# gt1/daccord

Measured on AMD Instinct MI355X. Metric: corrected Mbase/s (whole node), synthetic 20x PacBio piles, higher is better.
Workload: dtype u64+f64; 1 GPU; BASELINE.json configs[1] (10k A-reads x 10 kb x 20x, k=14, one MI355X): synthetic 10000 A-reads x 10000 b x 20x, 15% error (ins 80/del 13.3/sub 6.7), k=14, w=40, a=10, tspace=100; piles_total=10000, piles_rank0=10000, overlaps_rank0=319252, windows_rank0=9969965, trace_blocks_rank0=17906701, corrected_bases_total=90715992

## Files before the change

### daccord_amd/csrc/capi.hip

```cpp
#include <hip/hip_runtime.h>
#include <vector>
#include <string>
#include <cstring>
#include <cstdio>
#include <cstdlib>
#include <new>
#include "../../include/daccord_hip.h"
#include "batch_plan.hpp"
#include "host_tables.hpp"
#include "window_kernels.hpp"
#include "trace_kernel.hpp"
#include "vote_kernel.hpp"
#include "emit_record.hpp"
#include "context.hpp"

using namespace dacc;


struct PrepBatch
{
	DevOvl const * ovl; uint64_t novl; uint8_t const * trace; uint32_t trace_bytes;
	uint32_t * blk_ovl; uint32_t * blk_b0;
};

// ... 296 lines not shown
}

int dacc_create(dacc_ctx ** out, dacc_params const * p)
{
	if ( !out || !p ) return DACC_EINVAL;
	*out = 0;
	if ( p->klow < 3 || p->khigh > 16 || p->klow > p->khigh || !p->w || !p->a || p->w > DACC_WMAX || p->minfilterfreq < 0 ||
	     p->maxfilterfreq < p->minfilterfreq || p->tspace <= 0 || p->tspace > 512 )
		return DACC_EINVAL;
	if ( readTierSwitches().conflict() ) return DACC_EINVAL;
	int ndev = 0;
	if ( hipGetDeviceCount(&ndev) != hipSuccess || ndev <= 0 || p->device < 0 || p->device >= ndev )
		return DACC_ENODEV;
	if ( hipSetDevice(p->device) != hipSuccess ) return DACC_ENODEV;
	dacc_ctx * c = new (std::nothrow) dacc_ctx;
	if ( !c ) return DACC_ENOMEM;
	c->par = *p; c->device = p->device;
	c->sw = readTierSwitches();
	char const * sc = getenv("DACC_SCHED"); c->env_sched = sc ? atoi(sc) : 1;
	{ char const * td = getenv("DACC_TRACE_DYN"); c->env_trdyn = !(td && td[0] == '0'); }
	char const * ta = getenv("DACC_T7_ADAPT"); c->env_t7adapt = !(ta && ta[0] == '0');
	char const * dr = getenv("DACC_DEBUG_RETRY"); c->env_dbgretry = (dr && dr[0] == '1');
	{ char const * fn = getenv("DACC_FEAS_NEED"); c->env_feasneed = (fn && fn[0] == '0') ? 0u : 1u; }
	if ( hipStreamCreate(&c->stream.h) != hipSuccess ) { delete c; return DACC_EHIP; }
	{ int lo = 0, hi = 0; hipDeviceGetStreamPriorityRange(&lo,&hi); if ( hipStreamCreateWithPriority(&c->stream2.h,hipStreamNonBlocking,hi) != hipSuccess ) { delete c; return DACC_EHIP; } }
	hipEventCreateWithFlags(&c->evFirstTier.h,hipEventDisableTiming); hipEventCreateWithFlags(&c->evEarlyGeneric.h,hipEventDisableTiming); hipEventCreateWithFlags(&c->evPrescan.h,hipEventDisableTiming);
	for ( Event & e : c->ev ) hipEventCreate(&e.h);
	for ( Event & e : c->evEmit ) hipEventCreate(&e.h);
	for ( Event & e : c->evLong ) hipEventCreate(&e.h);
	for ( Event & e : c->evslot ) hipEventCreate(&e.h);
	for ( dacc_ctx::Stage & S : c->st ) hipEventCreate(&S.done.h);
	hipEventCreate(&c->h2dend.h);
	*out = c;
	return DACC_OK;
}

void dacc_destroy(dacc_ctx * c)
{
	if ( !c ) return;
	hipSetDevice(c->device);
	hipStreamSynchronize(c->stream); hipStreamSynchronize(c->stream2);
	delete c;
}

char const * dacc_last_error(dacc_ctx * c) { return c ? c->err.c_str() : "null context"; }

// ... 71 lines not shown
static uint32_t * workCounter(dacc_ctx * c, uint32_t const off) { return (c->sched&1) ? c->d_work.p+off : static_cast<uint32_t *>(0); }
static dacc_ctx::Stage * ranOf(dacc_ctx * c, TierId const id) { return c->st[id].ran ? &c->st[id] : static_cast<dacc_ctx::Stage *>(0); }

struct Pass
{
	WindowBatch WB;
	uint32_t const * list = 0;
	int lastslot = -1;
	bool early = false;
	uint32_t herr[4] = {0,0,0,0};
	size_t symbytes = 0;
};

static WindowBatch windowBatch(dacc_ctx * c)
{
	BatchPlan & BP = c->BP; WindowBatch WB;
	WB.P = c->P; WB.T = c->T; WB.C = BP.caps; WB.bps = c->d_bps.p; WB.boff = c->d_boff.p; WB.rlen = c->d_rlen.p;
	WB.piles = c->d_piles.p; WB.npiles = BP.piles.size(); WB.ovl = c->d_ovl.p; WB.wt_b = c->d_wt_b.p; WB.wt_e = c->d_wt_e.p;
	WB.nwindows = BP.nwindows; WB.wrec = c->d_wrec.p; WB.wout = c->d_wout.p; WB.arena = c->d_arena.p; WB.prof = c->d_prof.p;
	return WB;
}
static FastBatch stageBatch(dacc_ctx * c, WindowBatch const & WB, uint32_t const id, bool const chain = true)
{
	FastBatch FB; FB.W = WB; FB.F = c->BP.stageCaps(id); FB.dpsq_vst = c->d_vst.p; FB.tab32 = c->d_tab32.p; FB.feasneed = c->env_feasneed;
	if ( !chain ) return FB;
	FB.hand = c->handcap ? c->d_hand.p : static_cast<uint64_t *>(0); FB.handctr = c->d_handctr.p; FB.handcap = c->handcap; FB.handwords = c->TP.handwords;
#if defined(DACC_LEDGER)
	{ char const * lm = getenv("DACC_LEDGER_MASK"); FB.ledger = lm ? static_cast<uint32_t>(strtoul(lm,0,0)) : 0u; }
#endif
	return FB;
}
static void handsOn(FastBatch & FB, uint32_t * const handon, uint8_t * const slab) { FB.retry = handon; FB.gslab = slab; FB.gstride = FB.F.gbytes; }

static void growHandOver(dacc_ctx * c)
{
	if ( !(c->nruns && c->handwant > c->handcap && !c->nohand) ) return;
	uint64_t cap = c->handwant;
	{ size_t fr = 0, tot = 0; if ( hipMemGetInfo(&fr,&tot) == hipSuccess ) { uint64_t const lim = (static_cast<uint64_t>(fr)/2) / (static_cast<uint64_t>(c->TP.handwords)*8ull); if ( cap > lim ) cap = lim; } else (void)hipGetLastError(); }
	while ( cap && c->d_hand.ensure(static_cast<size_t>(cap)*c->TP.handwords) != hipSuccess ) { (void)hipGetLastError(); cap = cap > 65536 ? cap/2 : 0; }
	c->handcap = static_cast<uint32_t>(cap); c->handwant = cap;
}

static int enqueuePrepAndTrace(dacc_ctx * c)
{
	BatchPlan & BP = c->BP; hipStream_t const s = c->stream;
	HIPCHK(hipMemsetAsync(c->d_err.p,0,4*sizeof(uint32_t),s));
	HIPCHK(hipEventRecord(c->ev[0],s));
// ... 682 lines not shown
```

### daccord_amd/csrc/context.hpp

```cpp
#ifndef DACC_CONTEXT_HPP
#define DACC_CONTEXT_HPP
#include <hip/hip_runtime.h>
#include <cstdlib>
#include <string>
#include <vector>
#include "../../include/daccord_hip.h"
#include "batch_plan.hpp"
#include "host_tables.hpp"
#include "window_main.hpp"
#include "vote_kernel.hpp"

namespace dacc {

template<typename T>
struct DevBuf
{
	T * p = 0; size_t cap = 0;
	DevBuf() = default; DevBuf(DevBuf const &) = delete; DevBuf & operator=(DevBuf const &) = delete;
	~DevBuf() { release(); }
	hipError_t ensure(size_t n)
	{
		if ( n <= cap ) return hipSuccess;
		if ( p ) { hipFree(p); p = 0; cap = 0; }
		hipError_t const e = hipMalloc(reinterpret_cast<void **>(&p),n*sizeof(T));
// ... 52 lines not shown
	DevBuf<uint8_t> d_bps; DevBuf<uint64_t> d_boff; DevBuf<uint32_t> d_rlen;
	std::vector<uint32_t> h_rlen;
	BatchPlan BP;
	DevBuf<DevPile> d_piles; DevBuf<DevOvl> d_ovl; DevBuf<uint32_t> d_ovl_pile; DevBuf<uint8_t> d_trace;
	DevBuf<uint32_t> d_blk_ovl, d_blk_b0, d_wt_b, d_wt_e;
	DevBuf<uint8_t> d_wrec; DevBuf<WindowOut> d_wout; DevBuf<uint8_t> d_arena;
	DevBuf<uint8_t> d_has, d_oc, d_outsym, d_pilebad; DevBuf<uint16_t> d_ld0; DevBuf<uint32_t> d_ocs, d_nfrag, d_err;
	DevBuf<VoteFragment> d_frags; DevBuf<uint64_t> d_fragbase; DevBuf<uint64_t> d_prof;
	DevBuf<uint64_t> d_vst; DevBuf<uint32_t> d_tab32; DevBuf<uint8_t> d_gslab, d_arena2; DevBuf<uint64_t> d_trslab;
	DevBuf<uint32_t> d_retry[TIER_NSLOTS], d_work, d_gearly, d_pregen, d_pregen2, d_pregenlist, d_small;
	DevBuf<uint8_t> d_longslab;
	DevBuf<uint32_t> d_longhand[2];
	DevBuf<uint64_t> d_hand; DevBuf<uint32_t> d_handctr; uint32_t handcap = 0; uint64_t handwant = 0, nruns = 0; bool nohand = false, oom = false;
	bool noslab = false;
	bool tier7_adapt_off = false;
	TierSwitches sw = {}; TierPipeline TP = {};
	struct Stage { bool ran = false; uint32_t grid = 0; DevBuf<uint32_t> handon; DevBuf<uint8_t> slab; Event done; uint32_t const * in = 0;  } st[TIER_NROWS];
	uint32_t nlong[2] = {0,0};
	bool longran[2] = {false,false}; Event evLong[4];
	uint32_t retry_grid = 0, early_grid = 0; int sched = 0;
	uint32_t tr_grid = 0, tr_lds = 0, tr_words = 0, tr_lanes = 0, trace_bytes = 0, win_grid = 0;
	int env_sched = 1, env_dbgretry = 0, env_t7adapt = 1, env_trdyn = 1;
	uint32_t env_feasneed = 1;
	std::vector<uint32_t> retry_flags;
	std::vector<dacc_fragment> frags; std::string bases;
	std::vector<int32_t> pile_status; std::vector<std::string> pile_errors; std::string pile_errors_joined;
	std::vector<uint32_t> h_nfrag; std::vector<VoteFragment> h_frags; HostBuf<uint8_t> h_outsym;
	dacc_timing timing = {};
};

}

struct dacc_ctx : dacc::Context {};
#endif
```

### daccord_amd/csrc/fast_window.hpp

```cpp
#ifndef DACC_FAST_WINDOW_HPP
#define DACC_FAST_WINDOW_HPP
#include "wave.hpp"
#include "dev_types.hpp"
#include "arena.hpp"
#include "window_main.hpp"
#include "tier_pipeline.hpp"
#include "emit_record.hpp"

namespace dacc {

enum { WS_RETRY = 4 };
enum { FNOPAR = 0xFF };
enum { FSEQCAP = 48 };

struct FSI { uint64_t w; uint16_t left, right, current, path; };
struct FCC { uint64_t w; uint32_t o, l; };

template<int TIER> struct FastTier;
#if !defined(DACC_RCH01)
#define DACC_RCH01 2
#endif
template<> struct FastTier<1> { typedef uint8_t id_t; typedef uint8_t sid_t; enum : uint32_t { smax = 250, gw = 1, wcapg = 1024, rch = DACC_RCH01, fch = 4, fnw = 2, fnc = 40, idmax = 250, rpstcap = 256, lstr = 64, maxs = 32, precap = 1024, ncap = 776, scap = 112, lcap = 960, wcap = 1024, rccap = 144, fcap = 192, siqcap = 56, blcap = 96, seqcap = 32, psiq = 8, consrow = 64, lscrids = 2048, wide = 0, mins = 0, gmem = 0 }; };
template<> struct FastTier<0> { typedef uint8_t id_t; typedef uint8_t sid_t; enum : uint32_t { smax = 250, gw = 1, wcapg = 768, rch = DACC_RCH01, fch = 4, fnw = 2, fnc = 32, idmax = 250, rpstcap = 256, lstr = 64, maxs = 28, precap = 576, ncap = 524, scap = 88, lcap = 640, wcap = 768, rccap = 96, fcap = 128, siqcap = 56, blcap = 96, seqcap = 32, psiq = 8, consrow = 64, lscrids = 2048, wide = 0, mins = 0, gmem = 0 }; };
template<> struct FastTier<7> { typedef uint8_t id_t; typedef uint8_t sid_t; enum : uint32_t { smax = 250, gw = 1, wcapg = 896, rch = DACC_RCH01, fch = 4, fnw = 2, fnc = 32, idmax = 250, rpstcap = 256, lstr = 64, maxs = 28, precap = 704, ncap = 640, scap = 104, lcap = 800, wcap = 896, rccap = 112, fcap = 148, siqcap = 56, blcap = 96, seqcap = 32, psiq = 8, consrow = 64, lscrids = 2048, wide = 0, mins = 0, gmem = 0 }; };
// ... 401 lines not shown
	C.fcap = CT::fcap; C.siqcap = CT::siqcap; C.blcap = CT::blcap;
	C.nrows = nrows; C.nsup = nsup;
	C.ldsbytes = FastLds<CT>::bytes(nrows,nsup);
	C.tabcap = FastLds<CT>::tabcap;
	if constexpr ( CT::gw != 0 ) C.gbytes = FastLds<CT>::g_total; else C.gbytes = 0;
	if constexpr ( FastOneSlab<CT>::value != 0 ) C.ldsbytes = C.gbytes;
	C.gmem = CT::gmem;
	static_assert(CT::gmem == 0 || CT::gw != 0,"a layout in device memory is the gw layout");
	return C;
}

struct FastBatch
{
	WindowBatch W;
	FastCaps F = {};
	uint64_t const * dpsq_vst = 0;
	uint32_t * retry = 0;
	uint32_t * gearly = 0;
	uint8_t * gslab = 0;
	uint64_t gstride = 0;
	uint32_t const * tab32 = 0;
	uint64_t * hand = 0; uint32_t * handctr = 0; uint32_t handcap = 0, handwords = 0;
	uint32_t feasneed = 1;
#if defined(DACC_LEDGER)
	uint32_t ledger = 0;
#endif
};

template<typename CT>
DEV void fast_load_tables(FastLds<CT> const & L, uint32_t const nrows, uint32_t const nsup, DevTables const & T, uint64_t const * vst)
{
	int const lane = wv_lane();
	for ( uint32_t i = lane; i < nsup; i += WSZ ) { L.suplo8()[i] = T.suplo[i]; L.suphi8()[i] = T.suphi[i]; }
	wv_sync();
}

#if defined(DACC_LEDGER)
#define LEDGER_REP(bit) for ( uint32_t lrep_ = 0, lrn_ = 1u + ((ledger >> (bit)) & 1u); lrep_ < lrn_; ++lrep_ )
#define LEDGER_REPX(E,bit) for ( uint32_t lrep_ = 0, lrn_ = 1u + (((E).ledger >> (bit)) & 1u); lrep_ < lrn_; ++lrep_ )
#else
#define LEDGER_REP(bit)
#define LEDGER_REPX(E,bit)
#endif
#define FW_THRES_FEAS 4294968ull
#define FW_THRES_01   429496730ull
#define FW_THRES_05   2147483648ull

#if defined(DACC_EMUL)
struct FastStats { uint32_t v[32]; void clear() { for ( int i = 0; i < 32; ++i ) v[i] = 0; } void mx(int i, uint32_t x) { if ( x > v[i] ) v[i] = x; } void add(int i, uint32_t x) { v[i] += x; } };
static FastStats g_fstats;
static inline void fstats_dump(int const tier)
{
	static FILE * sf = 0; static bool tried = false;
	if ( !tried ) { tried = true; char const * fn = getenv("DACC_EMUL_STATS"); if ( fn ) sf = fopen(fn,"w"); }
	if ( sf ) { fprintf(sf,"%d",tier); for ( int i = 0; i < 32; ++i ) fprintf(sf," %u",g_fstats.v[i]); fprintf(sf,"\n"); fflush(sf); }
}
static inline FILE * ftrav_file() { static FILE * f = 0; static bool tried = false; if ( !tried ) { tried = true; char const * fn = getenv("DACC_EMUL_TRAV"); if ( fn ) f = fopen(fn,"w"); } return f; }
#define FSTAT_MX(i,x) g_fstats.mx(i,x)
#define FSTAT_ADD(i,x) g_fstats.add(i,x)
#include <vector>
#include <algorithm>
struct FeasIters { std::vector<uint32_t> it, ln; void clear() { it.clear(); ln.clear(); } };
static FeasIters g_feasit;
static inline void feasit_dump()
{
	static FILE * f = 0; static bool tried = false;
	if ( !tried ) { tried = true; char const * fn = getenv("DACC_EMUL_FEAS"); if ( fn ) f = fopen(fn,"w"); }
	if ( !f ) { g_feasit.clear(); return; }
	std::vector<uint32_t> const & it = g_feasit.it; std::vector<uint32_t> const & ln = g_feasit.ln;
	uint64_t tot = 0, lock = 0, locksorted = 0;
	for ( size_t i = 0; i < it.size(); ++i ) tot += it[i];
	for ( size_t i = 0; i < it.size(); i += 64 ) { uint32_t m = 0; for ( size_t q = i; q < it.size() && q < i+64; ++q ) m = std::max(m,it[q]); lock += m; }
	std::vector< std::pair<uint32_t,uint32_t> > P; for ( size_t i = 0; i < it.size(); ++i ) P.push_back(std::make_pair(ln[i],it[i]));
	std::stable_sort(P.begin(),P.end(),[](std::pair<uint32_t,uint32_t> const & a, std::pair<uint32_t,uint32_t> const & b){ return a.first > b.first; });
	for ( size_t i = 0; i < P.size(); i += 64 ) { uint32_t m = 0; for ( size_t q = i; q < P.size() && q < i+64; ++q ) m = std::max(m,P[q].second); locksorted += m; }
	uint64_t lockcls = 0;
	{
		std::vector< std::pair<uint32_t,uint32_t> > Q; for ( size_t i = 0; i < it.size(); ++i ) { uint32_t c = 0; while ( (2u<<c) <= ln[i] ) ++c; Q.push_back(std::make_pair(c,it[i])); }
// ... 111 lines not shown
template<typename CT>
struct FastEngine
{
	typedef typename CT::id_t id_t;
	typedef typename CT::sid_t sid_t;
	enum : uint32_t { SB = 8u*sizeof(sid_t), SMASK = (1u<<SB)-1u, SNONE = SMASK, SMAX = CT::smax };
	FastLds<CT> L; DevTables T; DevParams P;
	uint32_t nrows, nsup;
	uint64_t const * vst;
	enum : bool { GW = (CT::gw != 0) };
	uint8_t * gslab;
	uint32_t const * gtab;
	struct G4 { uint32_t x, y, z, w; };
	int lane; uint32_t flags;
#if defined(DACC_LEDGER)
	uint32_t ledger;
#endif
	uint64_t * prof;
	uint32_t mao, k; uint64_t kmask;
	uint32_t npre, nlast, nn, nmfirst, nmlast;
	uint32_t n0, npool, nlinks, nwF, nwR;
	uint32_t nF, nL;
	uint32_t feasneed;

#if defined(DACC_EMUL)
	bool feascount, feasapplied; uint32_t nwFall, nwRall;
	DEV bool feasNeedOn() const { char const * e = getenv("DACC_FEAS_NEED"); return !(e && e[0] == '0'); }
#else
	static constexpr bool feascount = false;
	DEV bool feasNeedOn() const { return feasneed != 0; }
#endif
#if defined(DACC_EMUL)
	DEV void over_(uint32_t b, int line) { flags |= b; static char const * ov = getenv("DACC_EMUL_OVER"); if ( ov ) fprintf(stderr,"[over] tier maxs=%d line %d bits 0x%x nn=%u n0=%u npool=%u nF=%u nL=%u nwF=%u nwR=%u rstop=%u\n",int(CT::maxs)*10000+int(CT::ncap),line,b,nn,n0,npool,nF,nL,nwF,nwR,rstop); }
	#define over(b) over_(b,__LINE__)
#else
	DEV void over(uint32_t b) { flags |= b; }
#endif
#if defined(DACC_PROFILE) && !defined(DACC_EMUL)
	DEV void pcount(int id, uint64_t v) { if ( prof ) atomicAdd(reinterpret_cast<unsigned long long *>(prof+id),static_cast<unsigned long long>(v)); }
	DEV uint64_t pclock() { return clock64(); }
#else
	DEV void pcount(int, uint64_t) {}
	DEV uint64_t pclock() { return 0; }
#endif

#if defined(DACC_PROFILE) && !defined(DACC_EMUL)
	#define SITE_T0 uint64_t _ps = clock64();
	#define SITE_RESET { _ps = clock64(); }
	#define SITE(id) { uint64_t const _n = clock64(); if ( prof && lane == static_cast<int>(__builtin_ctzll(__builtin_amdgcn_ballot_w64(true))) ) { atomicAdd(reinterpret_cast<unsigned long long *>(prof+32+(id)),static_cast<unsigned long long>(_n-_ps)); atomicAdd(reinterpret_cast<unsigned long long *>(prof+80+(id)),1ull); } _ps = clock64(); }
	#define PROFX_T0 uint64_t _px = clock64();
	#define PROFX(id) { uint64_t const _n = clock64(); if ( lane == 0 && prof ) atomicAdd(reinterpret_cast<unsigned long long *>(prof+(id)),static_cast<unsigned long long>(_n-_px)); _px = _n; }
#else
	#define PROFX_T0
// ... 594 lines not shown
			L.tlast()[q] = static_cast<uint32_t>(sk);
		}
		wv_sync();
		uint32_t const p2 = next_pow2(ns < 2 ? 2 : ns);
		for ( uint32_t q = lane; q < p2; q += WSZ )
		{
			if constexpr ( KEY2 ) L.skey()[q] = q < ns ? ((((static_cast<uint64_t>(L.tfirst()[q])<<KF) | L.links()[L.tlink()[q]+1])<<QB) | q) : ~0ull;
			else
			L.skey()[q] = q < ns ? ((sortKey(L.tfirst()[q],L.links()[L.tlink()[q]+1],L.tslen()[q] < KFMAX ? L.tslen()[q] : KFMAX,L.tlast()[q])<<QB) | q) : ~0ull;
		}
		wv_sync();
		wv_sort_keys<fcpow2(CT::scap)>(L.skey(),ns);
		uint32_t dup = 0;
		for ( uint32_t q = lane; q < ns; q += WSZ )
		{
			enum : uint32_t { DUPSH = KEY2 ? QB : QB+2*KF };
			if ( q && (L.skey()[q]>>DUPSH) == (L.skey()[q-1]>>DUPSH) ) dup = 1;
			uint32_t const raw = L.skey()[q]&QMASK;
			L.sfirst()[q] = L.tfirst()[raw]; L.slast()[q] = L.tlast()[raw]; L.sslen()[q] = L.tslen()[raw]; L.slink()[q] = L.tlink()[raw];
		}
		if ( wv_any(dup) ) { over(32); n0 = 0; return; }
		n0 = ns;
		wv_sync();
		for ( uint32_t z = lane; z < nn; z += WSZ ) { L.npred()[z] = SNONE; L.lhead()[z] = SNONE; }
		for ( uint32_t q = lane; q < p2; q += WSZ ) L.skey()[q] = q < ns ? ((static_cast<uint64_t>(L.slast()[q])<<SB) | q) : ~0ull;
		wv_sync();
		for ( uint32_t q = lane; q < ns; q += WSZ ) if ( q == 0 || L.sfirst()[q-1] != L.sfirst()[q] ) L.npred()[L.sfirst()[q]] = q;
		wv_sort_keys<fcpow2(CT::scap)>(L.skey(),ns);
		for ( uint32_t q = lane; q < ns; q += WSZ )
		{
			uint64_t const e = L.skey()[q];
			L.lord()[q] = static_cast<uint32_t>(e);
			if ( q == 0 || (L.skey()[q-1]>>SB) != (e>>SB) ) L.lhead()[e>>SB] = q;
		}
		wv_sync();
	}

	DEV void makePiece(uint32_t const id, uint32_t const par, uint32_t const a, uint32_t const b)
	{
		LDSQ uint16_t const * Lk = L.links() + L.slink()[par];
		L.sfirst()[id] = Lk[a]; L.slast()[id] = Lk[b]; L.sslen()[id] = b-a+1; L.slink()[id] = L.slink()[par]+a;
	}
	DEV void findCandidatesAndPieces()
	{
		uint32_t const firstthres = nmfirst ? ((static_cast<uint32_t>((~L.mfirst()[0])>>32))*3)/4 : 0;
		uint32_t const lastthres = nmlast ? ((static_cast<uint32_t>((~L.mlast()[0])>>32))*3)/4 : 0;
		uint32_t cf = 0, cl = 0;
		while ( cf < nmfirst && static_cast<uint32_t>((~L.mfirst()[cf])>>32) >= firstthres ) ++cf;
		while ( cl < nmlast && static_cast<uint32_t>((~L.mlast()[cl])>>32) >= lastthres ) ++cl;
		nF = cf; npool = n0;
		if ( nF > FNC ) { nL = cl; over(8); return; }
		for ( uint32_t i = lane; i < nF; i += WSZ ) { uint32_t const km = static_cast<uint32_t>(~L.mfirst()[i]); L.fkmer()[i] = km; int32_t const z = findNode(km); L.fnode()[i] = z < 0 ? 0xFFFF : z; L.parF()[i] = SNONE; L.pieF()[i] = SNONE; }
		{
			uint32_t nl = 0;
			for ( uint32_t c = 0; c < cl; c += WSZ )
			{
				uint32_t const i = c + lane;
				uint32_t const km = i < cl ? static_cast<uint32_t>(~L.mlast()[i]) : 0u;
// ... 14 lines not shown
			for ( uint32_t z = lane; z < nn; z += WSZ ) sid[z] = 0xFFFF;
			wv_sync();
			for ( uint32_t s = lane; s < n0; s += WSZ )
			{
				uint32_t const len = L.sslen()[s]; LDSQ uint16_t const * Lk = L.links() + L.slink()[s];
				for ( uint32_t i = len > 2 ? len-2 : 0; i >= 1; --i ) { uint32_t const z = Lk[i]; sid[z] = s; spos[z] = i; }
			}
			wv_sync();
			for ( uint32_t s = lane; s < n0; s += WSZ )
			{
				uint32_t const len = L.sslen()[s]; LDSQ uint16_t const * Lk = L.links() + L.slink()[s];
				for ( uint32_t i = 1; i+1 < len; ++i ) if ( sid[Lk[i]] != s ) multi = 1;
			}
			for ( uint32_t c = lane; c < nF; c += WSZ ) { uint32_t const z = L.fnode()[c]; if ( z != 0xFFFF && sid[z] != 0xFFFF ) { L.parF()[c] = sid[z]; L.posF()[c] = spos[z]; } }
			for ( uint32_t c = lane; c < nL; c += WSZ ) { uint32_t const z = L.lnode()[c]; if ( z != 0xFFFF && sid[z] != 0xFFFF ) { L.parL()[c] = sid[z]; L.posL()[c] = spos[z]; } }
		}
		if ( wv_any(multi) ) { over(32); return; }
		wv_sync();
		{
			uint32_t cnt = 0;
			for ( uint32_t c = 0; c < nF; ++c ) cnt += (L.parF()[c] != SNONE);
			for ( uint32_t c = 0; c < nL; ++c ) cnt += (L.parL()[c] != SNONE);
			if ( n0 + 2*cnt + 1 > CT::scap || n0 + 2*cnt + 1 > SMAX ) { over(32); return; }
		}
		{
			uint32_t id = n0;
			for ( uint32_t c0 = 0; c0 < nF + nL; c0 += WSZ )
			{
				uint32_t const c = c0 + lane;
				bool const isF = c < nF, act = c < nF + nL;
				uint32_t const ci = isF ? c : c - nF;
				uint32_t const par = act ? (isF ? L.parF()[ci] : L.parL()[ci]) : static_cast<uint32_t>(SNONE);
				bool const has = act && par != SNONE;
				uint32_t tot; uint32_t const pre = wv_scan_flag(has,tot);
				if ( has )
				{
					uint32_t const pid = id + 2*pre, pos = isF ? L.posF()[ci] : L.posL()[ci];
					if ( isF ) L.pieF()[ci] = pid; else L.pieL()[ci] = pid;
					makePiece(pid,par,0,pos); makePiece(pid+1,par,pos,L.sslen()[par]-1);
				}
				id += 2*tot;
			}
			npool = id;
		}
		wv_sync();
		nmid = 0; midbase = npool;
		{
			uint64_t pm = 0;
			for ( uint32_t c = lane; c < nF; c += WSZ ) { uint32_t const par = L.parF()[c]; if ( par != SNONE ) pm |= 1ull << (par & 63u); }
			pm = wv_or64(pm);
			uint32_t hit = 0;
			for ( uint32_t c = lane; c < nL; c += WSZ ) { uint32_t const par = L.parL()[c]; if ( par != SNONE && ((pm >> (par & 63u)) & 1ull) ) hit = 1; }
			if ( wv_any(hit) )
			{
				uint32_t nm = 0;
				if ( lane == 0 )
				{
					for ( uint32_t f = 0; f < nF && nm <= MIDCAP; ++f )
					{
						uint32_t const pf = L.parF()[f];
						if ( pf == SNONE ) continue;
						for ( uint32_t l = 0; l < nL && nm <= MIDCAP; ++l )
						{
							if ( L.parL()[l] != pf ) continue;
							uint32_t const a = L.posF()[f], b = L.posL()[l];
							if ( a == b ) continue;
							uint32_t const lo = a < b ? a : b, hi = a < b ? b : a;
							uint32_t m = 0;
							while ( m < nm && !(L.midpar()[m] == pf && L.midA()[m] == lo && L.midB()[m] == hi) ) ++m;
							if ( m < nm ) continue;
							if ( nm < MIDCAP ) { L.midpar()[nm] = pf; L.midA()[nm] = lo; L.midB()[nm] = hi; }
							++nm;
						}
					}
				}
				wv_sync();
				nm = wv_bcast(nm,0);
				if ( nm > MIDCAP || npool + nm > CT::scap || npool + nm > SMAX ) { over(32); return; }
				for ( uint32_t m = lane; m < nm; m += WSZ ) makePiece(npool+m,L.midpar()[m],L.midA()[m],L.midB()[m]);
				nmid = nm; npool += nm;
				wv_sync();
			}
		}
		for ( uint32_t id = n0 + lane; id < npool; id += WSZ ) L.ppos()[id] = basePos(id);
		wv_sync();

	}

	DEV bool pairReachable()
	{
		LDSQ uint8_t * const seedN = L.xreach();
		LDSQ uint8_t * const reachN = seedN + CT::ncap;
		LDSQ uint8_t * const vis = reachN + CT::ncap;
		if ( nF == 0 || nL == 0 ) return false;
		for ( uint32_t z = lane; z < nn; z += WSZ ) { seedN[z] = 0; reachN[z] = 0; }
		for ( uint32_t s = lane; s < n0; s += WSZ ) vis[s] = 0;
		wv_sync();
		for ( uint32_t c = lane; c < nF; c += WSZ )
		{
			uint32_t const z = L.fnode()[c], par = L.parF()[c];
			if ( z == 0xFFFF ) continue;
			if ( par == SNONE ) seedN[z] = 1; else reachN[L.slast()[par]] = 1;
		}
		wv_sync();
		while ( true )
		{
			uint32_t changed = 0;
			for ( uint32_t s = lane; s < n0; s += WSZ )
				if ( !vis[s] )
// ... 1858 lines not shown
		}
		return 0;
	}

	DEV bool traverse(int64_t const lmin, int64_t const lmax)
	{
		PROF_T0
		cfree = 0xFFFFu; ncdh = 0; nacc = 0; nwF = 0; nwR = 0; nsiq = 0; pvpath = pvrp = pvnf = 0; pvcl = ~0u;
		LEDGER_REP(5) computeBaseStretches();
		flags = wv_or(flags); if ( flags ) return false;
		PROF(*this,8)
		LEDGER_REP(6) findCandidatesAndPieces();
		flags = wv_or(flags); if ( flags ) return false;
		nLmagic = nL > 1 ? static_cast<uint32_t>(((1ull<<32) + nL - 1u) / nL) : 0u;
#if !defined(DACC_NO_REACH)
		{
			SITE_T0
			bool reach = false;
			LEDGER_REP(7) reach = pairReachable();
			SITE(23)
			if ( !reach ) { FSTAT_ADD(23,1); PROF(*this,16) return false; }
		}
#endif
		PROF(*this,16)
		loadTab();
		PROF(*this,17)
		LEDGER_REP(8) { nwF = 0; nwR = 0; bool const need = feasNeedOn(); if ( need ) feasDistances(); computeStretchFeasLanes(0,npool,lmax,need); }
		flags = wv_or(flags); if ( flags ) return false;
#if defined(DACC_EMUL)
		nwFall = nwF; nwRall = nwR;
		if ( ftrav_file() && feasapplied )
		{
			uint32_t const kF = nwF, kR = nwR;
			feascount = true; nwF = 0; nwR = 0; computeStretchFeasLanes(0,npool,lmax,false); feascount = false;
			nwFall = nwF; nwRall = nwR; nwF = kF; nwR = kR;
		}
#endif
		{ SITE_T0 bool const sf0_ = sfresh, sd0_ = sdirty; LEDGER_REP(9) { sfresh = sf0_; sdirty = sd0_; spillS(); } SITE(24) }
		PROF(*this,9)

		LEDGER_REP(10)
		{
		if ( lane == 0 ) { L.ctr()[0] = 0; L.ctr()[1] = 0; }
		wv_sync();
		{
			uint32_t sb = 0;
// ... 201 lines not shown
					wv_sync();
					flags = wv_bcast(flags,0); if ( flags ) return false;
					req = wv_bcast(req,0);
					if ( !req ) break;
					if ( req == 2 )
					{
						uint32_t const pq = p0 + wv_bcast(q,0);
						fstart += pq/nL; pskip = pq%nL; bw = 1; restart = true;
						if ( lane == 0 ) pcount(28,1);
						break;
					}
					break;
				}
				PROF(*this,7)
			}
			if ( restart ) continue;
			fstart += nb; pskip = 0;
		}
		{ SITE_T0 materializeKept(); SITE(34) }
		{ SITE_T0 LEDGER_REP(13) restoreS(); SITE(25) }
		PROF(*this,12)
		wv_sync();
		uint32_t const nkept = wv_bcast(ncdh,0);
		{
			uint32_t tie = 0;
			for ( uint32_t c = lane; c < nkept; c += WSZ )
			{
				FCC const e = ldget(L.cdh()+c);
				uint32_t rank = 0;
				for ( uint32_t j = 0; j < nkept; ++j ) { uint64_t const wj = L.cdh()[j].w; rank += (wj > e.w) ? 1u : 0u; tie |= (wj == e.w && j != c) ? 1u : 0u; }
				ldput(L.acc()+rank,e);
			}
			tie = wv_any(tie);
			FSTAT_ADD(21,tie ? 1u : 0u); FSTAT_ADD(22,nkept ? 1u : 0u);
			wv_sync();
			if ( lane == 0 )
			{
				if ( tie )
				{
					uint32_t nch = 0;
					while ( ncdh ) { FCC const c = ldget(L.cdh()); spop<FCC,true>(L.cdh(),ncdh); spush<FCC,false>(L.ch(),nch,c); }
					while ( nch ) { ldput(L.acc()+nacc,ldget(L.ch())); ++nacc; spop<FCC,false>(L.ch(),nch); }
				}
				else { nacc = nkept; ncdh = 0; }
			}
		}
		wv_sync();
		uint32_t const nc = wv_bcast(nacc,0);
		nacc = nc;
		for ( uint32_t c = lane; c < nc; c += WSZ )
		{
			uint32_t const slot = L.acc()[c].o, n = L.acc()[c].l & 0xFF;
			uint32_t const len = decodeSeq(L.cseq()+FSEQCAP*slot,n,L.consL()+c*CONSROW);
			L.acc()[c].o = c*CONSROW; L.acc()[c].l = len;
		}
		wv_sync();
		LEDGER_REP(14)
		for ( uint32_t t = lane; t < nc*mao; t += WSZ )
		{
			uint32_t const c = t / mao, j = t - c*mao;
			L.canderr()[t] = myersDistance(j,L.consL() + L.acc()[c].o,L.acc()[c].l);
		}
		wv_sync();
		for ( uint32_t c = lane; c < nc; c += WSZ )
		{
			uint32_t s = 0;
			for ( uint32_t j = 0; j < mao; ++j ) s += L.canderr()[c*mao+j];
			L.accerr()[c] = s;
		}
		wv_sync();
		{
			LDSQ uint32_t * const serr = reinterpret_cast<LDSQ uint32_t *>(L.canderr());
			static_assert(16*CT::maxs >= 64 && (FastLds<CT>::o_canderr & 3) == 0,"sorted error sums borrow the candidate error bytes");
			for ( uint32_t c = lane; c < nc; c += WSZ )
			{
				uint32_t const e = L.accerr()[c];
				uint32_t rank = 0;
				for ( uint32_t j = 0; j < nc; ++j ) { uint32_t const ej = L.accerr()[j]; rank += (ej < e || (ej == e && j < c)) ? 1u : 0u; }
				ldput(L.ch()+rank,ldget(L.acc()+c));
				serr[rank] = e;
			}
			wv_sync();
			for ( uint32_t c = lane; c < nc; c += WSZ ) { ldput(L.acc()+c,ldget(L.ch()+c)); L.accerr()[c] = serr[c]; }
		}
		wv_sync();
		PROF(*this,13)
		FSTAT_MX(0,mao); FSTAT_MX(1,npre); FSTAT_MX(2,nn); FSTAT_MX(3,n0); FSTAT_MX(4,npool); FSTAT_MX(5,nlinks); FSTAT_MX(6,nwF); FSTAT_MX(7,nwR);
		FSTAT_MX(8,rstop); FSTAT_MX(9,nF); FSTAT_MX(10,nL); FSTAT_ADD(11,1); FSTAT_MX(12,nc); FSTAT_ADD(24,nc ? 0u : 1u);
#if defined(DACC_EMUL)
		if ( lane == 0 ) { FILE * f = ftrav_file(); if ( f ) { uint32_t nlv = 0; for ( uint32_t i = 0; i < nL; ++i ) nlv += L.lnode()[i] != 0xFFFF; fprintf(f,"%d %u %u %u %u %u %u %u %u %u %u %u %u\n",int(CT::maxs),mao,npre,nn,n0,npool,nF,nL,nlv,rstop,nwFall,nwRall,nc); fflush(f); } }
#endif
		return nc != 0;
	}

	DEV int32_t estimateLength()
	{
		int32_t maxvprodindex = -1;
		uint32_t mn = 0xFFFFFFFFu, mx = 0;
		for ( uint32_t j = lane; j < mao; j += WSZ )
		{
			uint32_t const len = L.slen()[j];
			uint32_t const lastpos = len ? len-1 : 0;
			mn = lastpos < mn ? lastpos : mn; mx = lastpos > mx ? lastpos : mx;
		}
		mn = ~wv_max(~mn); mx = wv_max(mx);
		uint32_t const supStart = mn < static_cast<uint32_t>(T.nsup) ? T.suplo[mn] : T.nrows;
		uint32_t const supEnd = mx < static_cast<uint32_t>(T.nsup) ? T.suphi[mx] : T.nrows;
		uint64_t bestbits = 0; uint32_t besti = 0xFFFFFFFFu;
		for ( uint32_t c = supStart; c < supEnd; c += WSZ )
		{
			uint32_t const i = c + lane;
			double vprod = 0.0;
			if ( i < supEnd )
			{
				double const * row = T.dpnorm + static_cast<uint64_t>(i)*T.nsup;
// ... 181 lines not shown

template<typename CT>
DEV int processWindowFast(FastBatch const & FB, uint64_t const widx, LDSQ uint8_t * lds, bool const resume = false)
{
	WindowBatch const & B = FB.W;
	FastEngine<CT> E;
#if defined(DACC_EMUL)
	{ char const * pz = getenv("DACC_EMUL_POISON"); if ( pz ) __builtin_memset(static_cast<void *>(&E),atoi(pz),sizeof(E)); }
#endif
	if ( B.pregen && ((B.pregen[widx>>5] >> (widx&31)) & 1) ) return FW_DONE;
	E.mao = 0; E.k = 0; E.kmask = 0; E.npre = E.nlast = E.nn = E.nmfirst = E.nmlast = 0; E.n0 = E.npool = E.nlinks = E.nwF = E.nwR = 0; E.nF = E.nL = 0;
	E.nsiq = E.ncdh = E.nacc = 0; E.rstop = 0; E.roundT0 = 0; E.cfree = 0; E.pvpath = E.pvrp = E.pvnf = 0; E.pvcl = 0; E.nmid = 0; E.midbase = 0; E.nLmagic = 0;
	E.T = B.T; E.P = B.P; E.nrows = FB.F.nrows; E.nsup = FB.F.nsup; E.vst = FB.dpsq_vst;
	E.gslab = 0; E.gtab = FB.tab32; E.sfresh = true; E.sdirty = false;
	if ( CT::gw )
	{
#if defined(DACC_EMUL)
		E.gslab = FB.gslab;
#else
		E.gslab = FB.gslab + static_cast<uint64_t>(blockIdx.x)*FB.gstride;
#endif
		if constexpr ( FastOneSlab<CT>::value != 0 ) E.gslab = (uint8_t *)(lds) + FastLds<CT>::g_base;
	}
	E.lane = wv_lane(); E.flags = 0; E.prof = B.prof; E.feasneed = FB.feasneed;
#if defined(DACC_EMUL)
	E.feascount = false; E.feasapplied = false; E.nwFall = E.nwRall = 0;
#endif
#if defined(DACC_LEDGER)
	E.ledger = FB.ledger;
#endif
#if defined(DACC_PROFILE) && !defined(DACC_EMUL)
	uint64_t * const prof = E.prof;
#endif
#if defined(DACC_EMUL)
	g_fstats.clear();
#endif
	E.L.base = lds;
	FastLds<CT> const & L = E.L;
	int const lane = E.lane;
	PROF_T0
	int32_t curff = B.P.maxff;
	uint32_t hslot = 0;
	bool const handable = FB.hand != 0 && B.P.klow == B.P.khigh && CT::gw != 0;
	if ( resume && B.P.klow == B.P.khigh )
	{
		WindowOut const prev = B.wout[widx];
		if ( prev.status == WS_RETRY && prev.filterfreq <= B.P.maxff && prev.filterfreq >= B.P.minff )
// ... 240 lines not shown
```

Before: 41.81 Mbase/s.

## Skip serial heap ordering on weight ties unless top consensus is ambiguous

When candidate weights tie, the old code always fell back to a single-lane heap pop/push to order candidates. The new path resolves ties with a stable parallel rank sort, decodes and scores the candidates, and reruns the exact heap ordering only if the best candidate shares its error and weight with a different sequence. It also splits stretch-lookup and piece construction out of the pool builder into separate routines called later, after the reachability check. The cost is a possible second decode-and-score pass on ambiguous ties. The DACC_TIE_FAST switch, on by default, controls this.

Measured after the change: 42.64 Mbase/s, median of 6. 1.02x the previous value.

```diff
diff --git a/daccord_amd/csrc/capi.hip b/daccord_amd/csrc/capi.hip
--- a/daccord_amd/csrc/capi.hip
+++ b/daccord_amd/csrc/capi.hip
@@ -342,6 +342,7 @@
 	char const * ta = getenv("DACC_T7_ADAPT"); c->env_t7adapt = !(ta && ta[0] == '0');
 	char const * dr = getenv("DACC_DEBUG_RETRY"); c->env_dbgretry = (dr && dr[0] == '1');
 	{ char const * fn = getenv("DACC_FEAS_NEED"); c->env_feasneed = (fn && fn[0] == '0') ? 0u : 1u; }
+	{ char const * tf = getenv("DACC_TIE_FAST"); c->env_tiefast = (tf && tf[0] == '0') ? 0u : 1u; }
 	if ( hipStreamCreate(&c->stream.h) != hipSuccess ) { delete c; return DACC_EHIP; }
 	{ int lo = 0, hi = 0; hipDeviceGetStreamPriorityRange(&lo,&hi); if ( hipStreamCreateWithPriority(&c->stream2.h,hipStreamNonBlocking,hi) != hipSuccess ) { delete c; return DACC_EHIP; } }
 	hipEventCreateWithFlags(&c->evFirstTier.h,hipEventDisableTiming); hipEventCreateWithFlags(&c->evEarlyGeneric.h,hipEventDisableTiming); hipEventCreateWithFlags(&c->evPrescan.h,hipEventDisableTiming);
@@ -459,7 +460,7 @@
 }
 static FastBatch stageBatch(dacc_ctx * c, WindowBatch const & WB, uint32_t const id, bool const chain = true)
 {
-	FastBatch FB; FB.W = WB; FB.F = c->BP.stageCaps(id); FB.dpsq_vst = c->d_vst.p; FB.tab32 = c->d_tab32.p; FB.feasneed = c->env_feasneed;
+	FastBatch FB; FB.W = WB; FB.F = c->BP.stageCaps(id); FB.dpsq_vst = c->d_vst.p; FB.tab32 = c->d_tab32.p; FB.feasneed = c->env_feasneed; FB.tiefast = c->env_tiefast;
 	if ( !chain ) return FB;
 	FB.hand = c->handcap ? c->d_hand.p : static_cast<uint64_t *>(0); FB.handctr = c->d_handctr.p; FB.handcap = c->handcap; FB.handwords = c->TP.handwords;
 #if defined(DACC_LEDGER)
diff --git a/daccord_amd/csrc/context.hpp b/daccord_amd/csrc/context.hpp
--- a/daccord_amd/csrc/context.hpp
+++ b/daccord_amd/csrc/context.hpp
@@ -98,6 +98,7 @@
 	uint32_t tr_grid = 0, tr_lds = 0, tr_words = 0, tr_lanes = 0, trace_bytes = 0, win_grid = 0;
 	int env_sched = 1, env_dbgretry = 0, env_t7adapt = 1, env_trdyn = 1;
 	uint32_t env_feasneed = 1;
+	uint32_t env_tiefast = 1;
 	std::vector<uint32_t> retry_flags;
 	std::vector<dacc_fragment> frags; std::string bases;
 	std::vector<int32_t> pile_status; std::vector<std::string> pile_errors; std::string pile_errors_joined;
diff --git a/daccord_amd/csrc/fast_window.hpp b/daccord_amd/csrc/fast_window.hpp
--- a/daccord_amd/csrc/fast_window.hpp
+++ b/daccord_amd/csrc/fast_window.hpp
@@ -447,6 +447,7 @@
 	uint32_t const * tab32 = 0;
 	uint64_t * hand = 0; uint32_t * handctr = 0; uint32_t handcap = 0, handwords = 0;
 	uint32_t feasneed = 1;
+	uint32_t tiefast = 1;
 #if defined(DACC_LEDGER)
 	uint32_t ledger = 0;
 #endif
@@ -472,13 +473,13 @@
 #define FW_THRES_05   2147483648ull
 
 #if defined(DACC_EMUL)
-struct FastStats { uint32_t v[32]; void clear() { for ( int i = 0; i < 32; ++i ) v[i] = 0; } void mx(int i, uint32_t x) { if ( x > v[i] ) v[i] = x; } void add(int i, uint32_t x) { v[i] += x; } };
+struct FastStats { enum { N = 33 }; uint32_t v[N]; void clear() { for ( int i = 0; i < N; ++i ) v[i] = 0; } void mx(int i, uint32_t x) { if ( x > v[i] ) v[i] = x; } void add(int i, uint32_t x) { v[i] += x; } };
 static FastStats g_fstats;
 static inline void fstats_dump(int const tier)
 {
 	static FILE * sf = 0; static bool tried = false;
 	if ( !tried ) { tried = true; char const * fn = getenv("DACC_EMUL_STATS"); if ( fn ) sf = fopen(fn,"w"); }
-	if ( sf ) { fprintf(sf,"%d",tier); for ( int i = 0; i < 32; ++i ) fprintf(sf," %u",g_fstats.v[i]); fprintf(sf,"\n"); fflush(sf); }
+	if ( sf ) { fprintf(sf,"%d",tier); for ( int i = 0; i < FastStats::N; ++i ) fprintf(sf," %u",g_fstats.v[i]); fprintf(sf,"\n"); fflush(sf); }
 }
 static inline FILE * ftrav_file() { static FILE * f = 0; static bool tried = false; if ( !tried ) { tried = true; char const * fn = getenv("DACC_EMUL_TRAV"); if ( fn ) f = fopen(fn,"w"); } return f; }
 #define FSTAT_MX(i,x) g_fstats.mx(i,x)
@@ -636,13 +637,16 @@
 	uint32_t n0, npool, nlinks, nwF, nwR;
 	uint32_t nF, nL;
 	uint32_t feasneed;
+	uint32_t tiefast;
 
 #if defined(DACC_EMUL)
 	bool feascount, feasapplied; uint32_t nwFall, nwRall;
 	DEV bool feasNeedOn() const { char const * e = getenv("DACC_FEAS_NEED"); return !(e && e[0] == '0'); }
+	DEV bool tieFastOn() const { char const * e = getenv("DACC_TIE_FAST"); return !(e && e[0] == '0'); }
 #else
 	static constexpr bool feascount = false;
 	DEV bool feasNeedOn() const { return feasneed != 0; }
+	DEV bool tieFastOn() const { return tiefast != 0; }
 #endif
 #if defined(DACC_EMUL)
 	DEV void over_(uint32_t b, int line) { flags |= b; static char const * ov = getenv("DACC_EMUL_OVER"); if ( ov ) fprintf(stderr,"[over] tier maxs=%d line %d bits 0x%x nn=%u n0=%u npool=%u nF=%u nL=%u nwF=%u nwR=%u rstop=%u\n",int(CT::maxs)*10000+int(CT::ncap),line,b,nn,n0,npool,nF,nL,nwF,nwR,rstop); }
@@ -1283,6 +1287,12 @@
 		if ( wv_any(dup) ) { over(32); n0 = 0; return; }
 		n0 = ns;
 		wv_sync();
+	}
+	DEV void computeStretchLookups()
+	{
+		uint32_t const ns = n0, p2 = next_pow2(ns < 2 ? 2 : ns);
+		LEDGER_REP(20)
+		{
 		for ( uint32_t z = lane; z < nn; z += WSZ ) { L.npred()[z] = SNONE; L.lhead()[z] = SNONE; }
 		for ( uint32_t q = lane; q < p2; q += WSZ ) L.skey()[q] = q < ns ? ((static_cast<uint64_t>(L.slast()[q])<<SB) | q) : ~0ull;
 		wv_sync();
@@ -1295,6 +1305,7 @@
 			if ( q == 0 || (L.skey()[q-1]>>SB) != (e>>SB) ) L.lhead()[e>>SB] = q;
 		}
 		wv_sync();
+		}
 	}
 
 	DEV void makePiece(uint32_t const id, uint32_t const par, uint32_t const a, uint32_t const b)
@@ -1355,28 +1366,8 @@
 			for ( uint32_t c = 0; c < nF; ++c ) cnt += (L.parF()[c] != SNONE);
 			for ( uint32_t c = 0; c < nL; ++c ) cnt += (L.parL()[c] != SNONE);
 			if ( n0 + 2*cnt + 1 > CT::scap || n0 + 2*cnt + 1 > SMAX ) { over(32); return; }
-		}
-		{
-			uint32_t id = n0;
-			for ( uint32_t c0 = 0; c0 < nF + nL; c0 += WSZ )
-			{
-				uint32_t const c = c0 + lane;
-				bool const isF = c < nF, act = c < nF + nL;
-				uint32_t const ci = isF ? c : c - nF;
-				uint32_t const par = act ? (isF ? L.parF()[ci] : L.parL()[ci]) : static_cast<uint32_t>(SNONE);
-				bool const has = act && par != SNONE;
-				uint32_t tot; uint32_t const pre = wv_scan_flag(has,tot);
-				if ( has )
-				{
-					uint32_t const pid = id + 2*pre, pos = isF ? L.posF()[ci] : L.posL()[ci];
-					if ( isF ) L.pieF()[ci] = pid; else L.pieL()[ci] = pid;
-					makePiece(pid,par,0,pos); makePiece(pid+1,par,pos,L.sslen()[par]-1);
-				}
-				id += 2*tot;
-			}
-			npool = id;
-		}
-		wv_sync();
+			npool = n0 + 2*cnt;
+		}
 		nmid = 0; midbase = npool;
 		{
 			uint64_t pm = 0;
@@ -1410,14 +1401,39 @@
 				wv_sync();
 				nm = wv_bcast(nm,0);
 				if ( nm > MIDCAP || npool + nm > CT::scap || npool + nm > SMAX ) { over(32); return; }
-				for ( uint32_t m = lane; m < nm; m += WSZ ) makePiece(npool+m,L.midpar()[m],L.midA()[m],L.midB()[m]);
 				nmid = nm; npool += nm;
-				wv_sync();
-			}
-		}
+			}
+		}
+	}
+	DEV void makePieces()
+	{
+		LEDGER_REP(20)
+		{
+		{
+			uint32_t id = n0;
+			for ( uint32_t c0 = 0; c0 < nF + nL; c0 += WSZ )
+			{
+				uint32_t const c = c0 + lane;
+				bool const isF = c < nF, act = c < nF + nL;
+				uint32_t const ci = isF ? c : c - nF;
+				uint32_t const par = act ? (isF ? L.parF()[ci] : L.parL()[ci]) : static_cast<uint32_t>(SNONE);
+				bool const has = act && par != SNONE;
+				uint32_t tot; uint32_t const pre = wv_scan_flag(has,tot);
+				if ( has )
+				{
+					uint32_t const pid = id + 2*pre, pos = isF ? L.posF()[ci] : L.posL()[ci];
+					if ( isF ) L.pieF()[ci] = pid; else L.pieL()[ci] = pid;
+					makePiece(pid,par,0,pos); makePiece(pid+1,par,pos,L.sslen()[par]-1);
+				}
+				id += 2*tot;
+			}
+		}
+		wv_sync();
+		for ( uint32_t m = lane; m < nmid; m += WSZ ) makePiece(midbase+m,L.midpar()[m],L.midA()[m],L.midB()[m]);
+		wv_sync();
 		for ( uint32_t id = n0 + lane; id < npool; id += WSZ ) L.ppos()[id] = basePos(id);
 		wv_sync();
-
+		}
 	}
 
 	DEV bool pairReachable()
@@ -3322,6 +3338,8 @@
 			if ( !reach ) { FSTAT_ADD(23,1); PROF(*this,16) return false; }
 		}
 #endif
+		computeStretchLookups();
+		makePieces();
 		PROF(*this,16)
 		loadTab();
 		PROF(*this,17)
@@ -3569,75 +3587,118 @@
 		PROF(*this,12)
 		wv_sync();
 		uint32_t const nkept = wv_bcast(ncdh,0);
-		{
-			uint32_t tie = 0;
+		bool const tiefast = tieFastOn();
+		bool exact = false;
+		uint32_t tie = 0;
+		while ( true )
+		{
+			if ( !exact )
+			{
+				LEDGER_REP(18)
+				{
+				tie = 0;
+				for ( uint32_t c = lane; c < nkept; c += WSZ )
+				{
+					FCC const e = ldget(L.cdh()+c);
+					uint32_t rank = 0;
+					for ( uint32_t j = 0; j < nkept; ++j ) { uint64_t const wj = L.cdh()[j].w; rank += (wj > e.w || (wj == e.w && j < c)) ? 1u : 0u; tie |= (wj == e.w && j != c) ? 1u : 0u; }
+					ldput(L.acc()+rank,e);
+				}
+				tie = wv_any(tie);
+				}
+				FSTAT_ADD(21,tie ? 1u : 0u); FSTAT_ADD(22,nkept ? 1u : 0u);
+				if ( tie && !tiefast ) exact = true;
+				wv_sync();
+			}
+			if ( exact )
+			{
+#if defined(DACC_LEDGER)
+				FCC keep_[WSZ >= 16 ? 1 : 16]; for ( uint32_t c = lane; c < nkept; c += WSZ ) keep_[c/WSZ] = ldget(L.cdh()+c);
+#endif
+				LEDGER_REP(18)
+				{
+#if defined(DACC_LEDGER)
+				wv_sync(); for ( uint32_t c = lane; c < nkept; c += WSZ ) ldput(L.cdh()+c,keep_[c/WSZ]); wv_sync();
+#endif
+				if ( lane == 0 )
+				{
+					uint32_t nh = nkept, nch = 0, na = 0;
+					while ( nh ) { FCC const c = ldget(L.cdh()); spop<FCC,true>(L.cdh(),nh); spush<FCC,false>(L.ch(),nch,c); }
+					while ( nch ) { ldput(L.acc()+na,ldget(L.ch())); ++na; spop<FCC,false>(L.ch(),nch); }
+				}
+				}
+				if ( lane == 0 ) FSTAT_ADD(32,tiefast ? 1u : 0u);
+				wv_sync();
+			}
 			for ( uint32_t c = lane; c < nkept; c += WSZ )
 			{
-				FCC const e = ldget(L.cdh()+c);
-				uint32_t rank = 0;
-				for ( uint32_t j = 0; j < nkept; ++j ) { uint64_t const wj = L.cdh()[j].w; rank += (wj > e.w) ? 1u : 0u; tie |= (wj == e.w && j != c) ? 1u : 0u; }
-				ldput(L.acc()+rank,e);
-			}
-			tie = wv_any(tie);
-			FSTAT_ADD(21,tie ? 1u : 0u); FSTAT_ADD(22,nkept ? 1u : 0u);
+				uint32_t const slot = L.acc()[c].o, n = L.acc()[c].l & 0xFF;
+				uint32_t len = 0;
+				LEDGER_REP(19) len = decodeSeq(L.cseq()+FSEQCAP*slot,n,L.consL()+c*CONSROW);
+				L.acc()[c].o = c*CONSROW; L.acc()[c].l = len;
+			}
 			wv_sync();
-			if ( lane == 0 )
-			{
-				if ( tie )
-				{
-					uint32_t nch = 0;
-					while ( ncdh ) { FCC const c = ldget(L.cdh()); spop<FCC,true>(L.cdh(),ncdh); spush<FCC,false>(L.ch(),nch,c); }
-					while ( nch ) { ldput(L.acc()+nacc,ldget(L.ch())); ++nacc; spop<FCC,false>(L.ch(),nch); }
-				}
-				else { nacc = nkept; ncdh = 0; }
-			}
-		}
-		wv_sync();
-		uint32_t const nc = wv_bcast(nacc,0);
-		nacc = nc;
-		for ( uint32_t c = lane; c < nc; c += WSZ )
-		{
-			uint32_t const slot = L.acc()[c].o, n = L.acc()[c].l & 0xFF;
-			uint32_t const len = decodeSeq(L.cseq()+FSEQCAP*slot,n,L.consL()+c*CONSROW);
-			L.acc()[c].o = c*CONSROW; L.acc()[c].l = len;
-		}
-		wv_sync();
-		LEDGER_REP(14)
-		for ( uint32_t t = lane; t < nc*mao; t += WSZ )
-		{
-			uint32_t const c = t / mao, j = t - c*mao;
-			L.canderr()[t] = myersDistance(j,L.consL() + L.acc()[c].o,L.acc()[c].l);
-		}
-		wv_sync();
-		for ( uint32_t c = lane; c < nc; c += WSZ )
-		{
-			uint32_t s = 0;
-			for ( uint32_t j = 0; j < mao; ++j ) s += L.canderr()[c*mao+j];
-			L.accerr()[c] = s;
-		}
-		wv_sync();
-		{
-			LDSQ uint32_t * const serr = reinterpret_cast<LDSQ uint32_t *>(L.canderr());
-			static_assert(16*CT::maxs >= 64 && (FastLds<CT>::o_canderr & 3) == 0,"sorted error sums borrow the candidate error bytes");
-			for ( uint32_t c = lane; c < nc; c += WSZ )
-			{
-				uint32_t const e = L.accerr()[c];
-				uint32_t rank = 0;
-				for ( uint32_t j = 0; j < nc; ++j ) { uint32_t const ej = L.accerr()[j]; rank += (ej < e || (ej == e && j < c)) ? 1u : 0u; }
-				ldput(L.ch()+rank,ldget(L.acc()+c));
-				serr[rank] = e;
+			LEDGER_REP(14)
+			for ( uint32_t t = lane; t < nkept*mao; t += WSZ )
+			{
+				uint32_t const c = t / mao, j = t - c*mao;
+				L.canderr()[t] = myersDistance(j,L.consL() + L.acc()[c].o,L.acc()[c].l);
 			}
 			wv_sync();
-			for ( uint32_t c = lane; c < nc; c += WSZ ) { ldput(L.acc()+c,ldget(L.ch()+c)); L.accerr()[c] = serr[c]; }
-		}
-		wv_sync();
+			for ( uint32_t c = lane; c < nkept; c += WSZ )
+			{
+				uint32_t s = 0;
+				for ( uint32_t j = 0; j < mao; ++j ) s += L.canderr()[c*mao+j];
+				L.accerr()[c] = s;
+			}
+			wv_sync();
+			{
+				LDSQ uint32_t * const serr = reinterpret_cast<LDSQ uint32_t *>(L.canderr());
+				static_assert(16*CT::maxs >= 64 && (FastLds<CT>::o_canderr & 3) == 0,"sorted error sums borrow the candidate error bytes");
+				for ( uint32_t c = lane; c < nkept; c += WSZ )
+				{
+					uint32_t const e = L.accerr()[c];
+					uint32_t rank = 0;
+					for ( uint32_t j = 0; j < nkept; ++j ) { uint32_t const ej = L.accerr()[j]; rank += (ej < e || (ej == e && j < c)) ? 1u : 0u; }
+					ldput(L.ch()+rank,ldget(L.acc()+c));
+					serr[rank] = e;
+				}
+				wv_sync();
+				for ( uint32_t c = lane; c < nkept; c += WSZ ) { ldput(L.acc()+c,ldget(L.ch()+c)); L.accerr()[c] = serr[c]; }
+			}
+			wv_sync();
+			if ( exact || !tie ) break;
+			uint32_t amb = 0;
+			{
+				uint32_t const e0 = L.accerr()[0], l0 = L.acc()[0].l; uint64_t const w0 = L.acc()[0].w;
+				LDSQ uint64_t const * const r0 = reinterpret_cast<LDSQ uint64_t const *>(L.consL() + L.acc()[0].o);
+				for ( uint32_t c = lane; c < nkept; c += WSZ )
+					if ( c != 0 && L.accerr()[c] == e0 && L.acc()[c].w == w0 )
+					{
+						if ( L.acc()[c].l != l0 ) amb = 1;
+						else
+						{
+							LDSQ uint64_t const * const rc = reinterpret_cast<LDSQ uint64_t const *>(L.consL() + L.acc()[c].o);
+							uint64_t x = 0;
+							for ( uint32_t i = 0; i < (l0 >> 3); ++i ) x |= r0[i] ^ rc[i];
+							if ( l0 & 7u ) x |= (r0[l0 >> 3] ^ rc[l0 >> 3]) & ((1ull << (8u*(l0 & 7u))) - 1ull);
+							amb |= x ? 1u : 0u;
+						}
+					}
+			}
+			if ( !wv_any(amb) ) break;
+			exact = true;
+			wv_sync();
+		}
+		if ( lane == 0 ) ncdh = 0;
+		nacc = nkept;
 		PROF(*this,13)
 		FSTAT_MX(0,mao); FSTAT_MX(1,npre); FSTAT_MX(2,nn); FSTAT_MX(3,n0); FSTAT_MX(4,npool); FSTAT_MX(5,nlinks); FSTAT_MX(6,nwF); FSTAT_MX(7,nwR);
-		FSTAT_MX(8,rstop); FSTAT_MX(9,nF); FSTAT_MX(10,nL); FSTAT_ADD(11,1); FSTAT_MX(12,nc); FSTAT_ADD(24,nc ? 0u : 1u);
+		FSTAT_MX(8,rstop); FSTAT_MX(9,nF); FSTAT_MX(10,nL); FSTAT_ADD(11,1); FSTAT_MX(12,nkept); FSTAT_ADD(24,nkept ? 0u : 1u);
 #if defined(DACC_EMUL)
-		if ( lane == 0 ) { FILE * f = ftrav_file(); if ( f ) { uint32_t nlv = 0; for ( uint32_t i = 0; i < nL; ++i ) nlv += L.lnode()[i] != 0xFFFF; fprintf(f,"%d %u %u %u %u %u %u %u %u %u %u %u %u\n",int(CT::maxs),mao,npre,nn,n0,npool,nF,nL,nlv,rstop,nwFall,nwRall,nc); fflush(f); } }
+		if ( lane == 0 ) { FILE * f = ftrav_file(); if ( f ) { uint32_t nlv = 0; for ( uint32_t i = 0; i < nL; ++i ) nlv += L.lnode()[i] != 0xFFFF; fprintf(f,"%d %u %u %u %u %u %u %u %u %u %u %u %u\n",int(CT::maxs),mao,npre,nn,n0,npool,nF,nL,nlv,rstop,nwFall,nwRall,nkept); fflush(f); } }
 #endif
-		return nc != 0;
+		return nkept != 0;
 	}
 
 	DEV int32_t estimateLength()
@@ -3865,7 +3926,7 @@
 #endif
 		if constexpr ( FastOneSlab<CT>::value != 0 ) E.gslab = (uint8_t *)(lds) + FastLds<CT>::g_base;
 	}
-	E.lane = wv_lane(); E.flags = 0; E.prof = B.prof; E.feasneed = FB.feasneed;
+	E.lane = wv_lane(); E.flags = 0; E.prof = B.prof; E.feasneed = FB.feasneed; E.tiefast = FB.tiefast;
 #if defined(DACC_EMUL)
 	E.feascount = false; E.feasapplied = false; E.nwFall = E.nwRall = 0;
 #endif
```
